# Academich/translation-transformer

Hardware: AMD Instinct MI355X
Metric: reactions/sec (SMILES decoded), greedy speculative (higher is better)
Workload: dtype f32

## Files before the change

include/ttx.h:

```cpp
#ifndef TTX_H
#define TTX_H

#include <stdint.h>

#ifdef __cplusplus
extern "C" {
#endif

#define TTX_ABI_VERSION 4

typedef enum ttx_status {
  TTX_OK = 0,
  TTX_ERR_INVALID = -1,
  TTX_ERR_HIP = -2,
  TTX_ERR_NO_DEVICE = -3,
  TTX_ERR_REFERENCE = -4,
  TTX_ERR_NOMEM = -5,
  TTX_ERR_ROW_REPLAY = -6,
  TTX_ERR_MAX_STEPS = -7
} ttx_status;

typedef struct ttx_config {
  int32_t vocab_size;
  int32_t src_vocab_size;
// ... 490 lines not shown
  int32_t* d_row_of; int32_t* d_slot_batch; int32_t* d_src_acc; int32_t* d_src_state; int32_t* d_tok; int32_t* d_drafts_all;
  int32_t* d_bat_id; int32_t* d_bat_iter; int32_t* d_bat_dl; int32_t* d_bat_grp; int32_t* d_bat_live; int32_t* d_bat_nfin;
  int32_t* d_bat_longest_fin; int32_t* d_bat_longest_cur; int32_t* d_bat_state; int32_t* d_bat_given;
  int64_t* d_cand_next; int32_t* d_len_next; uint8_t* d_fin_next; float* d_logp_next; int32_t* d_parent; int32_t* d_parent_draft;
  int32_t* d_gen; int32_t* d_front; int32_t* d_len; uint8_t* d_active; uint8_t* d_finished; uint8_t* d_live; float* d_logp;
  int32_t* d_per_cand; int32_t* d_drafts32; int32_t* d_cand_dl; int32_t* d_cand_batch; int32_t* d_cache_slot; int32_t* d_cache_slot_parent;
  const int32_t* d_chosen_slot; const int64_t* d_chosen; const float* d_leaf_score; const int32_t* d_leaf_tok; const int32_t* d_leaf_cnt;
  int32_t* d_dev_summary;
  int64_t* d_out; int16_t* d_trace_len; int32_t* d_summary; const int32_t* d_len_all; const int32_t* d_batch_all; const int32_t* d_given_all;
  int32_t* d_src_of; int32_t* d_cand_src_len; int32_t* d_new_slot;
  const int32_t* d_tok_new; const uint8_t* d_valid_new; uint8_t* d_src_valid; const int32_t* d_drafts_new; float* d_memkv;
  const float* d_memkv_new;
  int32_t C, K, N, D0, Ls_cap, max_len, ld, smart, lib_ld, pad, bos, eos, repl, max_steps;
  int32_t T_cap, R, first_row, kv_row, Ls_new;
} ttx_debug_bsp_args;
int ttx_debug_bsp(ttx_session* s, int op, const ttx_debug_bsp_args* a, int64_t* words, void* stream);

int ttx_debug_kvcopy(ttx_session* s, const int32_t* d_rec, int n_copy, const float* d_qkv, int64_t qkv_layer_stride, float* d_kcache,
                     float* d_vcache, int64_t cache_layer_stride, int64_t cache_seq_stride, int N, int D, int d, int B, int Ld,
                     void* stream);

int ttx_debug_kvcopy_split(ttx_session* s, const int32_t* d_rec, int n_copy, const float* d_qkv, int64_t qkv_layer_stride,
                           float* d_kcache, float* d_vcache, int64_t cache_layer_stride, int64_t cache_seq_stride, int N, int D, int d,
                           int B, int Ld, const int32_t* d_pos2, const float* d_qkv_probe, int64_t probe_layer_stride, void* stream);

int ttx_debug_probe_split(ttx_session* s, const int32_t* d_act_idx, const int32_t* d_pred_probe, const int32_t* d_drafts, int B, int N,
                          int D, int n_active, int32_t* d_act2, int32_t* d_pos2, int32_t* result, void* stream);

int ttx_debug_merge_pred(ttx_session* s, const int32_t* d_pos2, const int32_t* d_pred_probe, const int32_t* d_pred2, int32_t* d_pred,
                         int B, int N, int D, int n_active, void* stream);

int ttx_debug_probe_split_select(ttx_session* s, const int32_t* d_act_idx, const int32_t* d_pred_probe, const int32_t* d_drafts, int B,
                                 int N, int D, int n_active, int32_t* d_act2, int32_t* d_pos2, int32_t* d_draft_mask, int32_t* d_row_base,
                                 int32_t* d_row_map, int32_t* result, void* stream);
int ttx_debug_merge_pred_select(ttx_session* s, const int32_t* d_pos2, const int32_t* d_pred_probe, const int32_t* d_pred2,
                                int32_t* d_pred, int B, int N, int D, int n_active, const int32_t* d_row_base,
                                const int32_t* d_draft_mask, void* stream);
int ttx_debug_kvcopy_select(ttx_session* s, const int32_t* d_rec, int n_copy, const float* d_qkv, int64_t qkv_layer_stride,
                            float* d_kcache, float* d_vcache, int64_t cache_layer_stride, int64_t cache_seq_stride, int N, int D, int d,
                            int B, int Ld, const int32_t* d_pos2, const float* d_qkv_probe, int64_t probe_layer_stride,
                            const int32_t* d_row_base, const int32_t* d_draft_mask, void* stream);
int ttx_debug_embed_select(ttx_session* s, const float* d_table, int V, const float* d_pe, int pe_rows, int d, float* d_x,
                           const int32_t* d_act_idx, const int32_t* d_front, const int32_t* d_gen, int gen_ld, const int32_t* d_drafts,
                           int B, int N, int D, int n_active, const int32_t* d_row_map, int m_rows, void* stream);
int ttx_debug_attn_select(ttx_session* s, const float* d_q, int ldq, const float* d_k, const float* d_v, int ldkv, float* d_out, int H,
                          float scale, int Lk, const int32_t* d_tok, int pad, const uint8_t* d_key_pad, const int32_t* d_act_idx,
                          const int32_t* d_front, const int32_t* d_src_of, const int32_t* d_src_len, const float* d_kcache,
                          const float* d_vcache, int64_t cache_seq_stride, const int32_t* d_cache_slot, int gen_ld, int N, int D, int mode,
                          int groups, int n_active, int max_keys, int kernel, int32_t* kernel_id, const int32_t* d_row_base,
                          const int32_t* d_draft_mask, void* stream);

int ttx_pool_last_counters(ttx_session* s, int64_t* counters);

int ttx_attn_staged_key_limit(int head_dim, int q_per_group);

int ttx_debug_attn_kernels_seen(ttx_session* s);

int ttx_debug_attn_probs(ttx_session* s, const float* d_q, int ldq, const float* d_k, int ldkv, const uint8_t* d_key_pad,
                         const int32_t* d_mem_row, const int32_t* d_length, int R, int Rm, int H, int head_dim, int T, int Ls,
                         float scale, float* d_heads, float* d_mean, int32_t* d_align, void* stream);

#ifdef __cplusplus
}
#endif
#endif
```

translation-transformer_amd/_native.py:

```python
from __future__ import annotations

import ctypes as C
import os
import subprocess
from pathlib import Path

PKG_DIR = Path(__file__).resolve().parent
CSRC = PKG_DIR / "csrc"
INCLUDE = PKG_DIR.parent / "include"
LIB_PATH = PKG_DIR / "libttx_hip.so"
UNITS = [CSRC / "ttx_api.hip", CSRC / "ttx_gemm.hip", CSRC / "ttx_attn.hip"]
HEADERS = [CSRC / "ttx_internal.h", CSRC / "ttx_common.hip.h", CSRC / "ttx_loop_kernels.hip.h", CSRC / "ttx_metrics.hip.h",
           CSRC / "ttx_score.hip.h", CSRC / "ttx_alternatives.hip.h", CSRC / "ttx_attn_probs.hip.h", CSRC / "ttx_sample.hip.h", CSRC / "ttx_logq.hip.h", CSRC / "ttx_sbs.hip.h", CSRC / "ttx_sbs_pool.hip.h",
           CSRC / "ttx_proposal.hip.h",
           CSRC / "ttx_select.h", CSRC / "ttx_tokenizer.h", CSRC / "ttx_drive.h", CSRC / "ttx_admit.h", INCLUDE / "ttx.h"]
SOURCES = UNITS + HEADERS
OBJ_DIR = CSRC / "build"

TTX_OK, TTX_ERR_INVALID, TTX_ERR_HIP, TTX_ERR_NO_DEVICE, TTX_ERR_REFERENCE, TTX_ERR_NOMEM = 0, -1, -2, -3, -4, -5
TTX_ERR_ROW_REPLAY = -6
TTX_ERR_MAX_STEPS = -7
TTX_ACT_NONE, TTX_ACT_RELU, TTX_ACT_GELU = 0, 1, 2
ACTIVATIONS = {"relu": TTX_ACT_RELU, "gelu": TTX_ACT_GELU}

# ... 275 lines not shown
                                 C.POINTER(C.c_int32), _VP]),
    "ttx_debug_gemm_act": (C.c_int, [_VP, _VP, _I, _VP, _I, _VP, _VP, _I, _VP, _I, _I, _I, _I, _I, C.c_int64, _I, _I,
                                     C.POINTER(C.c_int32), _VP]),
    "ttx_debug_finish_ln": (C.c_int, [_VP, _VP, _I, C.c_int64, _VP, _VP, _VP, _VP, _VP, _VP, _VP, _VP, _VP, _I, _I, C.c_float, _VP]),
    "ttx_debug_attn": (C.c_int, [_VP, _VP, _I, _VP, _VP, _I, _VP, _I, C.c_float, _I, _I, _VP, _I, _VP, _VP, _VP, _VP, _VP, _VP, _VP, _VP,
                                 C.c_int64, _VP, _I, _I, _I, _I, _I, _I, _I, _I, C.POINTER(C.c_int32), _VP]),
    "ttx_debug_attn_hd": (C.c_int, [_VP, _VP, _I, _VP, _VP, _I, _VP, _I, _I, C.c_float, _I, _I, _VP, _I, _VP, _VP, _VP, _VP, _VP, _VP, _VP,
                                    _VP, C.c_int64, _VP, _I, _I, _I, _I, _I, _I, _I, _I, C.POINTER(C.c_int32), _VP]),
    "ttx_debug_attn_as": (C.c_int, [_VP, _VP, _I, _VP, _VP, _I, _VP, _I, _I, C.c_float, _I, _I, _VP, _I, _VP, _VP, _VP, _VP, _VP, _VP, _VP,
                                    _VP, C.c_int64, _VP, _I, _I, _I, _I, _I, _I, _I, _I, C.POINTER(C.c_int32), _I, _I, _VP]),
    "ttx_debug_argmax": (C.c_int, [_VP, _VP, _I, _VP, _VP, _I, _VP]),
    "ttx_debug_sample": (C.c_int, [_VP, _VP, _I, _VP, _VP, _VP, _VP, _VP, _VP, _I, C.POINTER(SampleParams), _VP]),
    "ttx_debug_sample_step": (C.c_int, [_VP, _VP, _I, _VP, _VP, _VP, _VP, _I, _I, _I, _I, _VP, _VP, C.POINTER(SampleParams), _VP]),
    "ttx_debug_sample_accept": (C.c_int, [_VP, C.POINTER(DebugAcceptArgs), C.POINTER(C.c_int64), _VP]),
    "ttx_debug_sample_step_select": (C.c_int, [_VP, _VP, _I, _VP, _VP, _VP, _VP, _I, _I, _I, _I, _VP, _VP, C.POINTER(SampleParams),
                                              _VP, _I, _VP]),
    "ttx_debug_prefix_drafts": (C.c_int, [_VP, _VP, _VP, _I, _I, _I, _I, _VP, _VP, C.POINTER(DebugPrefix), _I, _I, _I, _VP]),
    "ttx_debug_proposal_drafts": (C.c_int, [_VP, _VP, _VP, _VP, _I, _I, _I, _I, _I, _VP, _VP, C.POINTER(DebugPrefix), _I, _I, _I, _I,
                                            _I, _VP]),
    "ttx_debug_sample_prefix": (C.c_int, [_VP, _VP, _I, _VP, _VP, _VP, _VP, _VP, _VP, _I, C.POINTER(SampleParams),
                                         C.POINTER(DebugPrefix), _VP]),
    "ttx_debug_sample_step_prefix": (C.c_int, [_VP, _VP, _I, _VP, _VP, _VP, _VP, _I, _I, _I, _I, _VP, _VP, C.POINTER(SampleParams),
                                              _VP, _I, C.POINTER(DebugPrefix), _VP]),
    "ttx_debug_sample_accept_pool": (C.c_int, [_VP, C.POINTER(DebugAcceptArgs), C.POINTER(C.c_int64), _VP, _I, _VP]),
    "ttx_debug_pool_fill_sample": (C.c_int, [_VP, C.POINTER(DebugPoolFillArgs), C.POINTER(C.c_int32), _VP]),
    "ttx_debug_embed": (C.c_int, [_VP, _VP, _I, _VP, _I, _I, _VP, _VP, _I, _I, _VP, _VP, _VP, _I, _VP, _I, _I, _I, _I, _I, _VP]),
    "ttx_debug_accept": (C.c_int, [_VP, C.POINTER(DebugAcceptArgs), C.POINTER(C.c_int64), _VP]),
    "ttx_debug_accept_block": (C.c_int, [_VP, C.POINTER(C.c_int32), _I, _VP]),
    "ttx_debug_bs_prep": (C.c_int, [_VP, C.POINTER(DebugBsPrepArgs), _VP]),
    "ttx_debug_bs_list": (C.c_int, [_VP, C.POINTER(DebugBsListArgs), C.POINTER(C.c_int64), _VP]),
    "ttx_debug_bs_hits": (C.c_int, [_VP, C.POINTER(DebugBsHitsArgs), _VP]),
    "ttx_debug_bs_leaves": (C.c_int, [_VP, C.POINTER(DebugBsLeavesArgs), _VP]),
    "ttx_debug_beam_select": (C.c_int, [_VP, C.POINTER(DebugBeamSelectArgs), _VP]),
    "ttx_debug_beam_step": (C.c_int, [_VP, C.POINTER(DebugBeamStepArgs), _VP]),
    "ttx_debug_sbs_step": (C.c_int, [_VP, C.POINTER(DebugSbsStepArgs), _VP]),
    "ttx_debug_sbs_step_ex": (C.c_int, [_VP, C.POINTER(DebugSbsStepArgs), _I, C.c_float, C.POINTER(DebugPrefix), _I, _VP]),
    "ttx_debug_sbs_step_pool": (C.c_int, [_VP, C.POINTER(DebugSbsStepPoolArgs), _I, _I, C.c_float, C.POINTER(DebugPrefix), _VP]),
    "ttx_debug_sbs_pool": (C.c_int, [_VP, _I, C.POINTER(DebugSbsPoolArgs), C.POINTER(C.c_int64), _VP]),
    "ttx_debug_tree_cache": (C.c_int, [_VP, C.POINTER(DebugTreeCacheArgs), _VP]),
    "ttx_debug_bsp": (C.c_int, [_VP, _I, C.POINTER(DebugBspArgs), C.POINTER(C.c_int64), _VP]),
    "ttx_debug_kvcopy": (C.c_int, [_VP, _VP, _I, _VP, C.c_int64, _VP, _VP, C.c_int64, C.c_int64, _I, _I, _I, _I, _I, _VP]),
    "ttx_debug_kvcopy_split": (C.c_int, [_VP, _VP, _I, _VP, C.c_int64, _VP, _VP, C.c_int64, C.c_int64, _I, _I, _I, _I, _I, _VP, _VP,
                                         C.c_int64, _VP]),
    "ttx_debug_probe_split": (C.c_int, [_VP, _VP, _VP, _VP, _I, _I, _I, _I, _VP, _VP, C.POINTER(C.c_int32), _VP]),
    "ttx_debug_merge_pred": (C.c_int, [_VP, _VP, _VP, _VP, _VP, _I, _I, _I, _I, _VP]),
    "ttx_debug_probe_split_select": (C.c_int, [_VP, _VP, _VP, _VP, _I, _I, _I, _I, _VP, _VP, _VP, _VP, _VP, C.POINTER(C.c_int32), _VP]),
    "ttx_debug_merge_pred_select": (C.c_int, [_VP, _VP, _VP, _VP, _VP, _I, _I, _I, _I, _VP, _VP, _VP]),
    "ttx_debug_kvcopy_select": (C.c_int, [_VP, _VP, _I, _VP, C.c_int64, _VP, _VP, C.c_int64, C.c_int64, _I, _I, _I, _I, _I, _VP, _VP,
                                          C.c_int64, _VP, _VP, _VP]),
    "ttx_debug_embed_select": (C.c_int, [_VP, _VP, _I, _VP, _I, _I, _VP, _VP, _VP, _VP, _I, _VP, _I, _I, _I, _I, _VP, _I, _VP]),
    "ttx_debug_attn_select": (C.c_int, [_VP, _VP, _I, _VP, _VP, _I, _VP, _I, C.c_float, _I, _VP, _I, _VP, _VP, _VP, _VP, _VP, _VP, _VP,
                                        C.c_int64, _VP, _I, _I, _I, _I, _I, _I, _I, _I, C.POINTER(C.c_int32), _VP, _VP, _VP]),
    "ttx_pool_last_counters": (C.c_int, [_VP, C.POINTER(C.c_int64)]),
    "ttx_attn_staged_key_limit": (C.c_int, [_I, _I]),
    "ttx_debug_attn_kernels_seen": (C.c_int, [_VP]),
    "ttx_last_kernel_profile": (C.c_int, [_VP, C.POINTER(C.c_double), C.POINTER(C.c_int64), C.POINTER(C.c_double)]),
}

_lib = None


def hipcc_path() -> str:
    for cand in (os.environ.get("HIPCC"), "/opt/rocm/bin/hipcc", "hipcc"):
        if cand and (os.path.isabs(cand) and os.path.exists(cand) or not os.path.isabs(cand)):
            return cand
    return "hipcc"


def needs_build() -> bool:
    if not LIB_PATH.exists():
        return True
    t = LIB_PATH.stat().st_mtime
    return any(src.stat().st_mtime > t for src in SOURCES)


def build(force: bool = False, verbose: bool = False) -> Path:
    if not force and not needs_build():
        return LIB_PATH
    OBJ_DIR.mkdir(exist_ok=True)
    flags = ["--offload-arch=gfx950", "-O3", "-std=c++17", "-fPIC", f"-I{INCLUDE}"] + os.environ.get("TTX_HIPCC_FLAGS", "").split()
    newest_header = max(h.stat().st_mtime for h in HEADERS)
    jobs, objs = [], []
    for unit in UNITS:
        obj = OBJ_DIR / (unit.stem + ".o")
        objs.append(str(obj))
        if not force and obj.exists() and obj.stat().st_mtime > max(unit.stat().st_mtime, newest_header) \
                and not os.environ.get("TTX_HIPCC_FLAGS"):
            continue
        cmd = [hipcc_path(), *flags, "-c", str(unit), "-o", str(obj)]
        if verbose:
            print(" ".join(cmd))
        jobs.append((cmd, subprocess.Popen(cmd)))
    for cmd, proc in jobs:
        if proc.wait() != 0:
            raise subprocess.CalledProcessError(proc.returncode, cmd)
    cmd = [hipcc_path(), "--offload-arch=gfx950", "-shared", "-fPIC", "-o", str(LIB_PATH), *objs]
    if verbose:
        print(" ".join(cmd))
    subprocess.run(cmd, check=True)
    return LIB_PATH


def lib():
    global _lib
    if _lib is not None:
        return _lib
# ... 23 lines not shown
```

translation-transformer_amd/csrc/ttx_admit.h:

```cpp
#pragma once
#include <algorithm>
#include <cstdint>
#include <vector>

namespace ttx {

inline int pool_slot_width(int len_max, int max_positions) {
  const int w = std::min(std::max(192, ((len_max + 63) / 64) * 64), max_positions);
  return std::max(w, std::max(2, len_max));
}

struct PoolShape { int n_jobs, C; };
inline PoolShape pool_shape(int n_sessions, int n_batches, int R_total, int capacity, int small_pool, int max_batch) {
  const int per_pool = std::max(1, std::min(capacity / 2, small_pool));
  const int n_jobs = std::max(1, std::min({n_sessions, n_batches, (R_total + per_pool - 1) / per_pool}));
  return {n_jobs, std::min(capacity, std::max(max_batch, (R_total + n_jobs - 1) / n_jobs))};
}

inline int serial_quota(const int* first, int n_batches, int cursor, int job, int n_jobs) {
  const int rest = first[n_batches] - first[cursor];
  const int target = first[cursor] + (rest + (n_jobs - job) - 1) / (n_jobs - job);
  int end = cursor;
  while (end < n_batches && first[end] < target) ++end;
  return end;
}

struct AdmitState {
  int cursor;
  int free_slots;
  int n_live;
  bool first_fill;
  int job, n_jobs;
  int n_running;
  bool serial;
  int quota_end;
};

inline int plan_admission(const int* first, int n_batches, int C, const AdmitState& a) {
  const int list_end = a.serial ? a.quota_end : n_batches;
  const int min_admit = std::max(1, C / 4);
  if (a.cursor >= list_end) return 0;
  if (a.n_live != 0 && a.free_slots < std::max(min_admit, first[a.cursor + 1] - first[a.cursor])) return 0;
  const int remaining = first[list_end] - first[a.cursor];
  const auto cdiv = [](int x, int y) { return (x + y - 1) / y; };
  int share = std::max(1, cdiv(remaining, std::max(1, a.serial ? 1 : a.n_running)));
  if (!a.serial && a.first_fill && (long long)a.n_jobs * C >= first[n_batches]) share = std::max(1, cdiv(remaining, a.n_jobs - a.job));
  int take = 0, end = a.cursor;
  while (end < list_end) {
    const int sz = first[end + 1] - first[end];
    if (take + sz > a.free_slots || (take > 0 && take + sz > share)) break;
    take += sz;
    ++end;
  }
  return end - a.cursor;
}

constexpr long long ADMIT_ROWS = 16384;
inline int chunk_width(const int32_t* len, int first, int end) {
  int w = 2;
  for (int r = first; r < end; ++r) w = std::max(w, (int)len[r]);
  return w;
}
inline void admit_chunks(const int32_t* len, int n, long long budget, std::vector<int>& ends) {
  ends.clear();
  if (budget > 0 && (long long)n * chunk_width(len, 0, n) >= budget) {
    int first = 0, w = 2;
    for (int r = 0; r < n; ++r) {
      w = std::max(w, (int)len[r]);
      if ((long long)(r + 1 - first) * w >= budget) { ends.push_back(r + 1); first = r + 1; w = 2; }
    }
    if (first < n) {
      const bool merge = !ends.empty() && (long long)(n - first) * chunk_width(len, first, n) * 2 < budget;
      if (merge) ends.back() = n; else ends.push_back(n);
    }
  } else {
    ends.push_back(n);
  }
}

}
```

translation-transformer_amd/csrc/ttx_api.hip:

```cpp
#include "ttx_internal.h"
#include "ttx_admit.h"
#include "ttx_drive.h"
#include "ttx_loop_kernels.hip.h"
#include "ttx_metrics.hip.h"
#include "ttx_score.hip.h"
#include "ttx_alternatives.hip.h"
#include "ttx_attn_probs.hip.h"
#include "ttx_sample.hip.h"
#include "ttx_logq.hip.h"
#include "ttx_sbs.hip.h"
#include "ttx_sbs_pool.hip.h"
#include "ttx_proposal.hip.h"
#include "ttx_tokenizer.h"

#include <algorithm>
#include <chrono>
#include <cmath>
#include <cstdio>
#include <cstdlib>
#include <cstring>
#include <mutex>
#include <type_traits>

using namespace ttx;
// ... 2036 lines not shown
  const int kcap = k.max_len;
  const int matches = ((volatile ProbeInfo*)s->probe_info)->matches;
  if (matches < 0 || matches > k.B) return fail(TTX_ERR_HIP, "slot pool: the probe published a match count outside the pool");
  const int RPS = step_rps(k.N, k.D);
  const long long rows = j.draft_select ? ((volatile ProbeInfo*)s->probe_info)->rows : (long long)matches * RPS;
  if (rows < (long long)matches * (matches ? 1 + k.D : 0) || rows > (long long)matches * RPS)
    return fail(TTX_ERR_HIP, "slot pool: the probe published a row count outside its matches' rows");
  DecState* st2 = s->state2.as<DecState>();
  k.st_ov = st2 + 1; k.act_ov = s->act2.as<int>(); k.pred_ov = s->pred_draft.as<int>();
  if (j.draft_select) { k.row_base = s->row_base.as<int>(); k.draft_mask = s->draft_mask.as<int>(); k.row_map = s->row_map.as<int>(); }
  k.variant = matches ? variant_for_rows(s, rows, true) : 0;
  j.matched_slot_steps += matches; j.skipped_draft_passes += matches ? 0 : 1;
  j.rows_executed += rows; j.drafts_matched += (rows - matches) / k.D;
  const int phase = j.draft_select ? (matches ? 5 : 6) : (matches ? 2 : 3);
  TTX_TRY(graph_replay(s, j.st, s->step_graphs, pool_key(j, k, k.variant, phase), [&]() -> int {
    if (matches) TTX_TRY(run_step(s, j.st, k, kcap));
    MergePredArgs mp{};
    mp.st = s->state.as<DecState>(); mp.pos2 = s->pos2.as<int>(); mp.pred_probe = s->pred_probe.as<int>();
    mp.pred2 = s->pred_draft.as<int>(); mp.pred = s->pred.as<int>(); mp.RPS = RPS;
    mp.row_base = k.row_base; mp.draft_mask = k.draft_mask; mp.D = k.D;
    hipLaunchKernelGGL(k_merge_pred, dim3(cdiv(k.B * RPS, 256)), dim3(256), 0, j.st, mp);
    HIP_TRY(hipGetLastError());
    return launch_accept_and_commit(s, j.st, j.g2, false);
  }));
  j.probe_pending = false;
  ++j.launched;
  return TTX_OK;
}

static int pool_sample_begin(PoolJob& j, const SampleSetup& smp) {
  ttx_session* s = j.s;
  hipLaunchKernelGGL(k_sample_params, dim3(1), dim3(64), 0, j.st, s->smp_prm.as<SampleBlock>(), smp.blk);
  HIP_TRY(hipGetLastError());
  StepCtx& k = j.g.k;
  k.want_sample_step = true;
  k.sample.key = s->smp_key.as<unsigned long long>(); k.sample.sample = s->smp_sample.as<unsigned>();
  k.sample.front = s->front.as<int>(); k.sample.prm = s->smp_prm.as<SampleBlock>();
  j.g.la.sample_rule = 1;
  j.per_src = smp.n; j.d_row_keys = smp.d_row_keys;
  if (smp.tabled()) {
    TTX_TRY(prefix_upload(s, j.st, smp, k.max_len, k.p.pad_token));
    const PrefixTab tab{s->pfx_tok.as<int>(), k.max_len, s->pfx_len.as<int>(), s->pfx_src.as<int>()};
    if (smp.proposed) { k.prop = tab; k.prop_ctx = smp.prop_ctx; }
    else k.sample.pfx = tab;
    k.pfx_draft0 = s->pfx_draft0.as<int>();
  }
  return TTX_OK;
}

static int pool_generate(ttx_session** sessions, int n_sessions, const int64_t* d_src, int R_total, int Ls_all, const int32_t* h_len,
                         int Ls_cap, int capacity, const ttx_gen_params* p, int64_t* d_out, int16_t* d_traj, int32_t* d_fin_step,
                         ttx_gen_stats* stats, void* stream, const SampleSetup* smp) {
  const int per = smp ? smp->n : 1;
  const PoolShape shape = pool_shape(n_sessions, R_total, R_total * per, capacity, 32, per);
  const int n_jobs = shape.n_jobs, C = shape.C;
  std::vector<int> first(R_total + 1);
  for (int r = 0; r <= R_total; ++r) first[r] = r * per;
  std::vector<PoolJob> jobs(n_jobs);
  std::vector<int> chunk_ends;
  std::fill(std::begin(sessions[0]->pool_counters), std::end(sessions[0]->pool_counters), 0LL);
  const bool serial = sessions[0]->profile;
  int cursor = 0;
  const auto start = [&](int i) -> int {
    TTX_TRY(pool_start(jobs[i], sessions[i], sessions[i]->own_stream, C, Ls_cap, p, d_out, d_traj, d_fin_step, smp));
    if (i == 0) sessions[0]->pool_counters[6] = jobs[0].draft_select ? 1 : 0;
    return TTX_OK;
  };
  const auto turn = [&](int i) -> int {
    PoolJob& j = jobs[i];
    ttx_session* s = j.s;
    volatile HostInfo* hi = s->host_info;
    if (j.phase == 1) {
      if (j.probe_pending) {
        if (((volatile ProbeInfo*)s->probe_info)->probes_done < j.probes) return TURN_WAITING;
        TTX_TRY(pool_launch_drafts(j));
        return TURN_PROGRESSED;
      }
      if (j.launched > 0 && hi->steps_done < j.launched) return TURN_WAITING;
      int n_act = (j.launched == 0) ? 0 : hi->n_active;
      if (serial && j.quota_end < 0) j.quota_end = serial_quota(first.data(), R_total, cursor, i, n_jobs);
      int n_running = 0;
      for (const PoolJob& o : jobs) n_running += (o.phase == 1);
      const int take = plan_admission(first.data(), R_total, C, {cursor, C - n_act, n_act, j.launched == 0, i, n_jobs, n_running, serial, j.quota_end});
      if (take > 0) {
        admit_chunks(h_len + cursor, take, j.admit_rows, chunk_ends);
        int r0 = cursor;
        for (const int end : chunk_ends) {
          const int r1 = cursor + end;
          TTX_TRY(pool_admit(j, d_src + (size_t)r0 * Ls_all, Ls_all, r1 - r0, chunk_width(h_len, r0, r1), r0, d_out, d_traj, d_fin_step));
          r0 = r1;
        }
        n_act += first[cursor + take] - first[cursor];
        cursor += take;
      }
      if (n_act == 0) {
        TTX_TRY(enqueue_readback(s, j.st, s->state.p, sizeof(DecState)));
        j.phase = 2;
      } else {
        if (j.launched > (long long)(p->max_len + 2) * (R_total + 1)) return fail(TTX_ERR_HIP, "decode loop failed to terminate");
        TTX_TRY(pool_launch_step(j, n_act));
      }
      return TURN_PROGRESSED;
    }
    if (hipEventQuery(s->ev_done) != hipSuccess) return TURN_IDLE;
    const DecState& hs = *s->host_state;
    if (stats) {
      add_counters(*stats, hs);
      stats->src_tokens_padded += j.src_tokens_padded;
      collect_gemm_profile(s, j.st);
      float ms = 0.f;
      if (hipEventElapsedTime(&ms, s->ev_a, s->ev_c) == hipSuccess) stats->decode_ms += ms;
    }
    if (getenv("TTX_TWO_PHASE_STATS"))
      fprintf(stderr, "[ttx two-phase] pool %d: %d steps, %lld split (%lld without a draft pass), %lld slot-steps probed, %lld matched, "
                      "%lld draft rows executed, %lld drafts matched\n",
              i, j.launched, j.split_steps, j.skipped_draft_passes, j.slot_steps, j.matched_slot_steps,
              j.rows_executed - j.slot_steps - j.unsplit_rows, j.drafts_matched);
    long long* pc = sessions[0]->pool_counters;
    pc[0] += j.launched; pc[1] += j.split_steps; pc[2] += j.slot_steps; pc[3] += j.matched_slot_steps;
    pc[4] += j.drafts_matched; pc[5] += j.rows_executed;
    j.phase = 3;
    if (hs.error == 3) return fail(TTX_ERR_ROW_REPLAY, "a row emitted PAD inside its sequence: decode the batches as given");
    if (hs.error) return fail(TTX_ERR_HIP, "slot pool bookkeeping failed (admitted more rows than free slots)");
    return TURN_FINISHED;
  };
  const int rc = drive_sessions(sessions, n_jobs, serial, stream, start, turn);
  if (stats) stats->status = rc;
  return rc;
}

extern "C" int ttx_greedy_speculative_generate_pool(ttx_session** sessions, int n_sessions, const int64_t* d_src, int R_total,
                                                    int Ls_all, const int32_t* h_len, int capacity, const ttx_gen_params* p,
                                                    int64_t* d_out, int16_t* d_traj, int32_t* d_fin_step, ttx_gen_stats* stats,
                                                    void* stream) {
  if (!sessions || n_sessions <= 0 || !d_src || R_total < 0 || !h_len || capacity <= 0 || capacity > 4096 || !p || !d_out || !d_traj ||
      !d_fin_step)
    return fail(TTX_ERR_INVALID, "bad argument to ttx_greedy_speculative_generate_pool");
  if (R_total == 0) return TTX_OK;
  if (p->max_len > 32000) return fail(TTX_ERR_INVALID, "max_len too large for the int16 trace");
  int len_max = 0;
  for (int i = 0; i < R_total; ++i) len_max = std::max(len_max, (int)h_len[i]);
  if (len_max > Ls_all) return fail(TTX_ERR_INVALID, "row length beyond the source matrix width");
  const int Ls_cap = pool_slot_width(len_max, sessions[0]->m->cfg.max_positions);
  TTX_TRY(gen_validate(sessions[0], d_src, capacity, Ls_cap, p, d_out, false));
  return pool_generate(sessions, n_sessions, d_src, R_total, Ls_all, h_len, Ls_cap, capacity, p, d_out, d_traj, d_fin_step, stats, stream,
                       nullptr);
// ... 2728 lines not shown
static int merge_pred_debug(ttx_session* s, const int32_t* d_pos2, const int32_t* d_pred_probe, const int32_t* d_pred2,
                            int32_t* d_pred, int B, int N, int D, int n_active, const int32_t* d_row_base, const int32_t* d_draft_mask,
                            void* stream) {
  hipStream_t st = reinterpret_cast<hipStream_t>(stream);
  if (!s || !d_pos2 || !d_pred_probe || !d_pred2 || !d_pred) return fail(TTX_ERR_INVALID, "null argument to ttx_debug_merge_pred");
  if (B < 1 || N < 1 || D < 1) return fail(TTX_ERR_INVALID, "ttx_debug_merge_pred: B, N and D must be positive");
  if (n_active < 0 || n_active > B) return fail(TTX_ERR_INVALID, "ttx_debug_merge_pred: n_active must lie in [0, B]");
  HIP_TRY(hipSetDevice(s->m->device));
  HIP_TRY(hipStreamSynchronize(st));
  if (n_active > 0) {
    std::vector<int> pos((size_t)n_active);
    HIP_TRY(hipMemcpy(pos.data(), d_pos2, (size_t)n_active * 4, hipMemcpyDeviceToHost));
    for (int p : pos)
      if (p < -1 || p >= B) return fail(TTX_ERR_INVALID, "ttx_debug_merge_pred: pos2 must lie in [-1, B)");
    if (d_row_base || d_draft_mask) {
      int n_pos = 0, total = 0;
      for (int p : pos) n_pos = std::max(n_pos, p + 1);
      TTX_TRY(dbg_check_select("ttx_debug_merge_pred_select", d_row_base, d_draft_mask, n_pos, N, D, st, nullptr, &total));
    }
  }
  DecState* dst = nullptr;
  TTX_TRY(dbg_state_with(st, n_active, 0, &dst));
  MergePredArgs mp{};
  mp.st = dst; mp.pos2 = d_pos2; mp.pred_probe = d_pred_probe; mp.pred2 = d_pred2; mp.pred = d_pred; mp.RPS = step_rps(N, D);
  mp.row_base = d_row_base; mp.draft_mask = d_draft_mask; mp.D = D;
  hipLaunchKernelGGL(k_merge_pred, dim3(cdiv(B * mp.RPS, 256)), dim3(256), 0, st, mp);
  hipError_t err = hipGetLastError();
  const hipError_t esync = hipStreamSynchronize(st);
  (void)hipFree(dst);
  HIP_TRY(err);
  HIP_TRY(esync);
  return TTX_OK;
}

extern "C" int ttx_debug_merge_pred(ttx_session* s, const int32_t* d_pos2, const int32_t* d_pred_probe, const int32_t* d_pred2,
                                    int32_t* d_pred, int B, int N, int D, int n_active, void* stream) {
  return merge_pred_debug(s, d_pos2, d_pred_probe, d_pred2, d_pred, B, N, D, n_active, nullptr, nullptr, stream);
}

extern "C" int ttx_debug_merge_pred_select(ttx_session* s, const int32_t* d_pos2, const int32_t* d_pred_probe, const int32_t* d_pred2,
                                           int32_t* d_pred, int B, int N, int D, int n_active, const int32_t* d_row_base,
                                           const int32_t* d_draft_mask, void* stream) {
  if ((d_row_base != nullptr) != (d_draft_mask != nullptr))
    return fail(TTX_ERR_INVALID, "ttx_debug_merge_pred_select: row_base and draft_mask come together");
  return merge_pred_debug(s, d_pos2, d_pred_probe, d_pred2, d_pred, B, N, D, n_active, d_row_base, d_draft_mask, stream);
}

extern "C" int ttx_pool_last_counters(ttx_session* s, int64_t* counters) {
  if (!s || !counters) return fail(TTX_ERR_INVALID, "null argument to ttx_pool_last_counters");
  for (int i = 0; i < 7; ++i) counters[i] = s->pool_counters[i];
  return TTX_OK;
}

extern "C" int ttx_attn_staged_key_limit(int head_dim, int q_per_group) { return attn_staged_key_limit(head_dim, q_per_group); }

extern "C" int ttx_debug_attn_kernels_seen(ttx_session* s) {
  if (!s) return fail(TTX_ERR_INVALID, "null session");
  return (int)s->attn_kernels_seen;
}

extern "C" int ttx_last_kernel_profile(ttx_session* s, double* gemm_ms, int64_t* gemm_launches, double* empty_pair_ms) {
  if (!s) return fail(TTX_ERR_INVALID, "null session");
  if (gemm_ms) *gemm_ms = s->prof_ms;
  if (gemm_launches) *gemm_launches = s->prof_launches;
  s->prof_ms = 0;
  s->prof_launches = 0;
  if (empty_pair_ms) *empty_pair_ms = s->prof_empty_pair_ms < 0 ? 0.0 : s->prof_empty_pair_ms;
  return TTX_OK;
}
```

translation-transformer_amd/csrc/ttx_internal.h:

```cpp
#pragma once
#include "ttx.h"
#include "ttx_common.hip.h"

#include <map>
#include <set>
#include <string>
#include <utility>
#include <vector>

namespace ttx {
struct BeamHost;
struct BeamPoolHost;
}

struct LayerW {
  size_t sa_in_w, sa_in_b, sa_out_w, sa_out_b;
  size_t ca_in_w, ca_in_b, ca_out_w, ca_out_b;
  size_t l1_w, l1_b, l2_w, l2_b;
  size_t n1_w, n1_b, n2_w, n2_b, n3_w, n3_b;
};

struct ttx_model {
  ttx_config cfg;
  int device;
// ... 52 lines not shown
  X(ev_logits) X(ev_pred) X(ev_nll)                                                                                              \
   \
                                                                                                      \
  X(sc_src_of) X(am_length)                                                                                                                   \
                                    \
  X(lq_tok)                                                                                                                      \
                                                                                                                       \
  X(drafts) X(gen) X(front) X(act_idx) X(rec) X(pred) X(state) X(kcache) X(vcache) X(src32) X(outbuf) X(haspad) X(traj)           \
  X(fin_step)                                                                                                                    \
                                                                                            \
  X(rstep) X(row_of) X(src_len) X(new_slot) X(pool_io) X(memkv_new) X(valid_new) X(drafts_new)                                    \
       \
            \
  X(qkv_probe) X(pred_probe) X(pred_draft) X(act2) X(pos2) X(state2)                                                             \
         \
  X(draft_mask) X(row_base) X(row_map)                                                                                           \
                           \
  X(accept_blk)                                                                                                                  \
                                        \
  X(snap_logits) X(snap_act) X(snap_front) X(snap_gen) X(snap_state)                                                             \
  X(leaf_score) X(leaf_tok) X(leaf_cnt) X(beam_summary)                                                                          \
                                                                                               \
  X(bs_cand_next) X(bs_len_next) X(bs_fin_next) X(bs_logp_next) X(bs_len) X(bs_fin) X(bs_active) X(bs_logp) X(bs_per_cand)        \
  X(bs_best_n) X(bs_best_slot) X(bs_chosen) X(bs_parent) X(bs_parent_draft) X(bs_mark) X(bs_drafts_src) X(bs_cnt) X(bs_hit)       \
                                                                                 \
  X(t_prev_len) X(t_slot_of) X(t_src_of)                                                                                         \
                                            \
  X(bp_row_of) X(bp_batch) X(bp_cand) X(bp_cand_len) X(bp_tok) X(bp_new_slot) X(bp_io) X(bp_grp) X(bp_src_acc) X(bp_enc_qkv)            \
   \
                     \
  X(smp_key) X(smp_sample) X(smp_done) X(smp_src_of) X(smp_prm) X(smp_drafts)                                                     \
   \
       \
  X(pfx_tok) X(pfx_len_src) X(pfx_len) X(pfx_src) X(pfx_draft0)                                                                  \
    \
  X(sbs_g) X(sbs_g_next)                                                                                                         \
   \
                                                                                          \
  X(sbp_slot) X(sbp_len) X(sbp_io)
#define TTX_DECLARE_BUF(name) Buf name;
#define TTX_REGISTER_BUF(name) all.push_back(&name);

#ifndef TTX_BIG_MIN_TILES
#define TTX_BIG_MIN_TILES 400
#endif
struct ttx_session {
  ttx_model* m;
  std::vector<Buf*> all;
  TTX_SESSION_BUFS(TTX_DECLARE_BUF)
  Buf tk[2], tv[2];
  int snap_B = 0, snap_rps = 0, snap_gen_ld = 0, snap_step = 0;
  ttx::ProbeInfo* probe_info = nullptr;
  long long pool_counters[7] = {};
  ttx::BeamHost* beam_host = nullptr;
  ttx::BeamPoolHost* bp_host = nullptr;
  ttx::HostInfo* host_info = nullptr;
  hipStream_t own_stream = nullptr;
  uint64_t alloc_generation = 0;
  uint64_t graphs_generation = 0;
  bool dead = false;
  bool use_graphs = true;
  GraphCache step_graphs{512};
  GraphCache iter_graphs{256};
  hipEvent_t ev_done = nullptr;
  void drop_graphs() { step_graphs.clear(); iter_graphs.clear(); }
  void graphs_current() { if (graphs_generation != alloc_generation) { drop_graphs(); graphs_generation = alloc_generation; } }
  ttx::DecState* host_state = nullptr;
  bool attr_attn2[2][8] = {};
  bool attr_select = false, attr_step = false, attr_topk = false, attr_pool_select = false, attr_sbs_step = false;
  bool attr_sbs_step_masked[5] = {};
  bool attr_sbs_step_pool = false, attr_sbs_step_pool_masked[5] = {};
  bool attr_attn_probs[8] = {};
  int qkv_small_rows = 800;
  int small_rows = 2000;
  int ffn2_slab_rows = 5600;
  int big_min_tiles = TTX_BIG_MIN_TILES;
  int last_gemm_kernel = 0, last_gemm_big_min_tiles = 0;
  int attn_split = -1;
  int attn_row = -1;
  bool accept_spread = true;
  bool attn_fallback = false;
  int attn_force = 0;
  int attn_sel_N = 0, attn_sel_D = 0;
  int last_attn_kernel = 0;
  unsigned attn_kernels_seen = 0;
  bool profile = false;
  std::vector<std::pair<hipEvent_t, hipEvent_t>> ev_pool;
  size_t ev_used = 0;
  double prof_ms = 0;
  double prof_empty_pair_ms = -1;
  long long prof_launches = 0;
  bool host_timing = false;
  double host_launch_us = 0;
  long long host_captures = 0;
  double host_capture_us = 0;
  long long host_launches = 0;
  hipEvent_t ev_a = nullptr, ev_b = nullptr, ev_c = nullptr;
  ttx_session() {
    TTX_SESSION_BUFS(TTX_REGISTER_BUF)
    for (Buf* b : {&tk[0], &tk[1], &tv[0], &tv[1]}) all.push_back(b);
    for (Buf* b : all) b->owner_gen = &alloc_generation;
  }
};

namespace ttx {

// ... 45 lines not shown
```

translation-transformer_amd/decoding.py:

```python
from __future__ import annotations

import ctypes as C
import os
from typing import NamedTuple

import numpy as np
import torch

from . import _native as N
from .model import AttentionMaps, HypothesisScores, NativeTransformer, ProposalScores


def _need_native(model) -> NativeTransformer:
    if not isinstance(model, NativeTransformer):
        raise TypeError("the native generators run on a NativeTransformer (no eager/PyTorch fallback exists)")
    return model


class _ScoresHypotheses:

    def _pad_eos(self) -> tuple:
        return self.pad_token, self.eos_token

    def score(self, src: torch.Tensor, pred: torch.Tensor, **kw) -> HypothesisScores:
# ... 121 lines not shown
            return []
        if reorder:
            try:
                if pool is None:
                    pool = True
                return self._generate_reordered(batches, in_flight, group_size, on_error, pool)
            except N.TtxError as e:
                if e.code != N.TTX_ERR_ROW_REPLAY:
                    raise
        srcs = [b.to(m.device, torch.int64).contiguous() for b in batches]
        for b in srcs:
            m.check_tokens(b)
        outs = [torch.empty((s.shape[0], 1, self.max_len), dtype=torch.int64, device=m.device) for s in srcs]
        n = len(srcs)
        pool = m.session_pool(max(1, min(in_flight, n)))
        sess = (C.c_void_p * len(pool))(*[p.value for p in pool])
        src_p = (C.c_void_p * n)(*[s.data_ptr() for s in srcs])
        out_p = (C.c_void_p * n)(*[o.data_ptr() for o in outs])
        Bs = (C.c_int * n)(*[s.shape[0] for s in srcs])
        Ls = (C.c_int * n)(*[s.shape[1] for s in srcs])
        p = N.GenParams(self.max_len, self.draft_len, self.n_drafts, self.pad_token, self.bos_token, self.eos_token,
                        self.replace_token, 0)
        stats = (N.GenStats * n)()
        rc = m._lib.ttx_greedy_speculative_generate_many(sess, len(pool), n, src_p, Bs, Ls, C.byref(p), out_p, stats, m._stream())
        if not (rc == N.TTX_ERR_REFERENCE and on_error == "skip"):
            N.check(rc)
        t = self.stats_total
        for i, st in enumerate(stats):
            if st.status != N.TTX_OK:
                if st.status != N.TTX_ERR_REFERENCE:
                    N.check(int(st.status))
                outs[i] = None
                self.last_failed_batches.append(i)
                continue
            self.model_calls_num += int(st.model_calls)
            self.last_batch_counters[i] = {"model_calls_num": int(st.model_calls)}
            for k in ("accepted_tokens", "produced_tokens", "verified_positions", "kv_prefix_positions", "src_positions",
                      "encode_ms", "decode_ms"):
                t[k] += getattr(st, k)
            t["src_tokens_padded"] += srcs[i].shape[0] * srcs[i].shape[1]
            t["batches"] += 1
        return outs

    def _generate_reordered(self, batches: list, in_flight: int, group_size: int | None, on_error: str = "raise",
                            pool: bool = True) -> list:
        from .scheduling import plan_row_groups, replay_batch
        m = self.model
        L, T = self.max_len, self.max_len + 1
        srcs = [b.to(m.device, torch.int64) for b in batches]
        sizes = [int(s.shape[0]) for s in srcs]
        R = sum(sizes)
        if pool:
            gsz, pool_sessions = _slot_pool_plan(R, in_flight, group_size)
        else:
            gsz = int(group_size or min(256, max(max(sizes), -(-R // max(1, in_flight)))))
        self.last_group_size = gsz
        Lmax = max(int(s.shape[1]) for s in srcs)
        allsrc = torch.full((R, Lmax), self.pad_token, dtype=torch.int64, device=m.device)
        r0 = 0
        for s in srcs:
            allsrc[r0:r0 + s.shape[0], :s.shape[1]] = s
            r0 += s.shape[0]
        m.check_tokens(allsrc)
        pos = torch.arange(1, Lmax + 1, device=m.device)
        lengths = ((allsrc != self.pad_token) * pos).amax(dim=1)
        order, groups = plan_row_groups(lengths.cpu().numpy(), gsz)
        order_t = torch.from_numpy(order).to(m.device)
        sorted_src = allsrc[order_t]
        sorted_len = lengths[order_t].cpu().numpy()
        out_sorted = torch.empty((R, L), dtype=torch.int64, device=m.device)
        traj_sorted = torch.empty((R, T), dtype=torch.int16, device=m.device)
        fin_sorted = torch.empty((R,), dtype=torch.int32, device=m.device)
        p = N.GenParams(L, self.draft_len, self.n_drafts, self.pad_token, self.bos_token, self.eos_token, self.replace_token, 0)
        if pool:
            sessions = m.session_pool(pool_sessions)
            sess = (C.c_void_p * len(sessions))(*[q.value for q in sessions])
            width = max(2, int(sorted_len.max()))
            src_mat = sorted_src[:, :width].contiguous() if width <= sorted_src.shape[1] else torch.nn.functional.pad(
                sorted_src, (0, width - sorted_src.shape[1]), value=self.pad_token).contiguous()
            h_len = (C.c_int32 * R)(*[int(x) for x in sorted_len])
            one = N.GenStats()
            N.check(m._lib.ttx_greedy_speculative_generate_pool(sess, len(sessions), src_mat.data_ptr(), R, width, h_len, gsz,
                                                                C.byref(p), out_sorted.data_ptr(), traj_sorted.data_ptr(),
                                                                fin_sorted.data_ptr(), C.byref(one), m._stream()))
            stats, gsrc = [one], [src_mat]
        else:
            gsrc = [sorted_src[g, :max(2, int(sorted_len[g].max()))].contiguous() for g in groups]
            n = len(gsrc)
            sessions = m.session_pool(max(1, min(in_flight, n)))
            sess = (C.c_void_p * len(sessions))(*[q.value for q in sessions])
            src_p = (C.c_void_p * n)(*[s.data_ptr() for s in gsrc])
            out_p = (C.c_void_p * n)(*[out_sorted[g].data_ptr() for g in groups])
            traj_p = (C.c_void_p * n)(*[traj_sorted[g].data_ptr() for g in groups])
            fin_p = (C.c_void_p * n)(*[fin_sorted[g].data_ptr() for g in groups])
            Bs = (C.c_int * n)(*[s.shape[0] for s in gsrc])
            Ls = (C.c_int * n)(*[s.shape[1] for s in gsrc])
            stats = (N.GenStats * n)()
            N.check(m._lib.ttx_greedy_speculative_generate_rows(sess, len(sessions), n, src_p, Bs, Ls, C.byref(p), out_p, traj_p, fin_p,
                                                                stats, m._stream()))
        inv = torch.empty_like(order_t)
        inv[order_t] = torch.arange(R, device=m.device)
        out_rows = out_sorted[inv]
        traj = traj_sorted[inv].cpu().numpy()
        fin = fin_sorted[inv].cpu().numpy()
        keep = torch.zeros(R, dtype=torch.bool)
        t = self.stats_total
        failed = None
        r0 = 0
        for bi, B in enumerate(sizes):
            rep = replay_batch(traj[r0:r0 + B], fin[r0:r0 + B], L, self.draft_len, self.n_drafts)
            if rep.error:
                if on_error == "skip":
                    self.last_failed_batches.append(bi)
                    r0 += B
                    continue
                failed = bi
                break
            keep[r0:r0 + B] = torch.from_numpy(rep.finished)
            self.model_calls_num += rep.model_calls
            self.last_batch_counters[bi] = {"model_calls_num": rep.model_calls}
            t["accepted_tokens"] += rep.accepted_tokens
            t["produced_tokens"] += rep.produced_tokens
            t["verified_positions"] += rep.verified_positions
            t["kv_prefix_positions"] += rep.kv_prefix_positions
            t["src_positions"] += rep.rows_iterations * int(srcs[bi].shape[1])
            t["src_tokens_padded"] += B * int(srcs[bi].shape[1])
            t["batches"] += 1
            r0 += B
        for st in stats:
            t["encode_ms"] += st.encode_ms
            t["decode_ms"] += st.decode_ms
        dv = t.setdefault("device", {"model_calls": 0, "accepted_tokens": 0, "produced_tokens": 0, "verified_positions": 0,
                                     "kv_prefix_positions": 0, "src_positions": 0, "src_tokens_padded": 0, "batches": 0})
        for st, gs in zip(stats, gsrc):
            for k in ("model_calls", "accepted_tokens", "produced_tokens", "verified_positions", "kv_prefix_positions",
                      "src_positions"):
                dv[k] += int(getattr(st, k))
            dv["src_tokens_padded"] += int(st.src_tokens_padded) if pool else int(gs.numel())
            dv["batches"] += 1
        t["device_model_calls"] = dv["model_calls"]
        if failed is not None:
            raise N.ReferenceError_(f"batch {failed}: a row finished at a width beyond max_len: shape mismatch in the reference "
                                    "(speculative_decoding.py:158)")
        out_rows = torch.where(keep.to(m.device)[:, None], out_rows, torch.full_like(out_rows, self.pad_token))
        outs, r0 = [], 0
        skipped = set(self.last_failed_batches)
        for bi, B in enumerate(sizes):
            outs.append(None if bi in skipped else out_rows[r0:r0 + B].unsqueeze(1).contiguous())
            r0 += B
        return outs


class TranslationInferenceGreedy(_ScoresHypotheses):

    def __init__(self, model, max_len: int, pad_token: int, bos_token: int, eos_token: int) -> None:
        self.model = _need_native(model)
        self.max_len = max_len
# ... 703 lines not shown
```

translation-transformer_amd/model.py:

```python
from __future__ import annotations

import ctypes as C
import os
import math
from typing import NamedTuple

import numpy as np
import torch

from . import _native as N


def reference_pe_table(emb: int, max_len: int = 5000) -> torch.Tensor:
    pe = torch.zeros(max_len, emb)
    position = torch.arange(0, max_len, dtype=torch.float).unsqueeze(1)
    div_term = torch.exp(torch.arange(0, emb, 2).float() * (-math.log(10000.0) / emb))
    pe[:, 0::2] = torch.sin(position * div_term)
    pe[:, 1::2] = torch.cos(position * div_term)
    return torch.vstack((torch.zeros(1, emb), pe)).contiguous()


def _strip(state: dict) -> dict:
    if any(k.startswith("model.") for k in state):
        return {k[len("model."):]: v for k, v in state.items() if k.startswith("model.")}
# ... 531 lines not shown
                                n: int, d: int, n_active: int, row_base: torch.Tensor | None, draft_mask: torch.Tensor | None) -> None:
        N.check(self._lib.ttx_debug_merge_pred_select(self._session, pos2.data_ptr(), pred_probe.data_ptr(), pred2.data_ptr(),
                                                      pred.data_ptr(), int(B), int(n), int(d), int(n_active), self._ptr(row_base),
                                                      self._ptr(draft_mask), self._stream()))

    def debug_kvcopy_select(self, rec: torch.Tensor, n_copy: int, qkv: torch.Tensor, kcache: torch.Tensor, vcache: torch.Tensor,
                            n: int, d: int, width: int, B: int, pos2: torch.Tensor | None, qkv_probe: torch.Tensor | None,
                            row_base: torch.Tensor | None, draft_mask: torch.Tensor | None) -> None:
        assert kcache.stride() == vcache.stride()
        N.check(self._lib.ttx_debug_kvcopy_select(self._session, rec.data_ptr(), int(n_copy), qkv.data_ptr(), int(qkv.stride(0)),
                                                  kcache.data_ptr(), vcache.data_ptr(), int(kcache.stride(0)), int(kcache.stride(1)),
                                                  int(n), int(d), int(width), int(B), int(qkv.shape[0]), self._ptr(pos2),
                                                  self._ptr(qkv_probe), 0 if qkv_probe is None else int(qkv_probe.stride(0)),
                                                  self._ptr(row_base), self._ptr(draft_mask), self._stream()))

    def debug_embed_select(self, table: torch.Tensor, pe: torch.Tensor, x: torch.Tensor, act_idx: torch.Tensor, front: torch.Tensor,
                           gen: torch.Tensor, drafts: torch.Tensor, B: int, n: int, d: int, n_active: int,
                           row_map: torch.Tensor | None, m_rows: int) -> None:
        N.check(self._lib.ttx_debug_embed_select(self._session, table.data_ptr(), int(table.shape[0]), pe.data_ptr(), int(pe.shape[0]),
                                                 int(table.shape[1]), x.data_ptr(), act_idx.data_ptr(), front.data_ptr(),
                                                 gen.data_ptr(), int(gen.stride(0)), drafts.data_ptr(), int(B), int(n), int(d),
                                                 int(n_active), self._ptr(row_map), int(m_rows), self._stream()))

    def debug_attn_select(self, mode: int, q: torch.Tensor, k: torch.Tensor, v: torch.Tensor, out: torch.Tensor, heads: int,
                          scale: float, groups: int, max_keys: int, row_base: torch.Tensor | None, draft_mask: torch.Tensor | None,
                          Lk: int = 0, tok: torch.Tensor | None = None, pad: int = 0, key_pad: torch.Tensor | None = None,
                          act_idx: torch.Tensor | None = None, front: torch.Tensor | None = None, src_of: torch.Tensor | None = None,
                          src_len: torch.Tensor | None = None, kcache: torch.Tensor | None = None, vcache: torch.Tensor | None = None,
                          cache_seq_stride: int = 0, cache_slot: torch.Tensor | None = None, gen_ld: int = 0, n: int = 1, d: int = 0,
                          n_active: int = 0, kernel: int = 0, **unused) -> int:
        kid = C.c_int32(0)
        assert k.stride(0) == v.stride(0)
        N.check(self._lib.ttx_debug_attn_select(self._session, q.data_ptr(), q.stride(0), k.data_ptr(), v.data_ptr(), k.stride(0),
                                                out.data_ptr(), int(heads), float(scale), int(Lk), self._ptr(tok), int(pad),
                                                self._ptr(key_pad), self._ptr(act_idx), self._ptr(front), self._ptr(src_of),
                                                self._ptr(src_len), self._ptr(kcache), self._ptr(vcache), int(cache_seq_stride),
                                                self._ptr(cache_slot), int(gen_ld), int(n), int(d), int(mode), int(groups),
                                                int(n_active), int(max_keys), int(kernel), C.byref(kid), self._ptr(row_base),
                                                self._ptr(draft_mask), self._stream()))
        return int(kid.value)

    def attn_kernels_seen(self, session=None) -> set:
        mask = int(self._lib.ttx_debug_attn_kernels_seen(self._session if session is None else session))
        if mask < 0:
            N.check(mask)
        return {k for k in range(1, 32) if mask >> k & 1}

    POOL_COUNTERS = ("steps", "split_steps", "slot_steps_probed", "slots_matched", "drafts_matched", "rows_executed", "draft_select")

    def pool_last_counters(self, session=None) -> dict:
        words = (C.c_int64 * 7)()
        N.check(self._lib.ttx_pool_last_counters(self._session if session is None else session, words))
        return dict(zip(self.POOL_COUNTERS, (int(v) for v in words)))

    @staticmethod
    def attn_staged_key_limit(head_dim: int, q_per_group: int) -> int:
        return int(N.lib().ttx_attn_staged_key_limit(int(head_dim), int(q_per_group)))

    def close(self) -> None:
        if getattr(self, "_score_session", None):
            self._lib.ttx_session_destroy(self._score_session)
            self._score_session = None
        for extra in getattr(self, "_pool", [])[1:]:
            self._lib.ttx_session_destroy(extra)
        self._pool = None
        if getattr(self, "_session", None):
            self._lib.ttx_session_destroy(self._session)
            self._session = None
        if getattr(self, "_model", None):
            self._lib.ttx_model_destroy(self._model)
            self._model = None

    def __del__(self):
        try:
            self.close()
        except Exception:
            pass

    def _tokens(self, t: torch.Tensor) -> torch.Tensor:
        return t.to(self.device, torch.int64).contiguous()

    def check_tokens(self, t: torch.Tensor, vocab: int | None = None) -> None:
        if t.numel() == 0:
            return
        lo, hi = int(t.min()), int(t.max())
        if lo < 0 or hi >= (vocab or self.src_vocab_size):
            raise IndexError("index out of range in self")

    def encode_src(self, src: torch.Tensor, src_pad_mask: torch.Tensor | None = None) -> torch.Tensor:
        src = self._tokens(src)
        self.check_tokens(src)
        B, Ls = src.shape
        mem = torch.empty((B, Ls, self.emb_dim), dtype=torch.float32, device=self.device)
        N.check(self._lib.ttx_encode_src(self._session, src.data_ptr(), B, Ls, mem.data_ptr(), self._stream()))
        return mem

    def decode_tgt(self, tgt: torch.Tensor, memory: torch.Tensor, memory_pad_mask: torch.Tensor,
                   memory_row: torch.Tensor | None = None) -> torch.Tensor:
        tgt = self._tokens(tgt)
        R, Lt = tgt.shape
        memory = memory.to(self.device, torch.float32).contiguous()
        Rm, Ls, _ = memory.shape
        pad = memory_pad_mask.to(self.device, torch.uint8).contiguous()
        row_ptr = None
        if memory_row is not None:
            memory_row = memory_row.to(self.device, torch.int32).contiguous()
# ... 366 lines not shown
```

Baseline: 23880.

## Add dedicated head pool job that decodes the first rows alongside bulk pools

Adds a separate head session that takes the first H rows, by default three quarters of the capacity, in a single admission. The remaining rows are spread over the bulk pool jobs, and the Python planner adds one extra pool session when the head plan applies. The aim is to start work on the leading rows straight away and keep the device busy while bulk jobs run, which should improve overlap and load balance. It costs one more concurrent session, changes admission accounting, and adds layout introspection APIs.

```diff
diff --git a/include/ttx.h b/include/ttx.h
--- a/include/ttx.h
+++ b/include/ttx.h
@@ -566,6 +566,10 @@
 
 int ttx_pool_last_counters(ttx_session* s, int64_t* counters);
 
+int ttx_pool_last_layout(ttx_session* s, int32_t* words);
+
+int ttx_head_pool_rows(int n_sessions, int rows_total, int capacity);
+
 int ttx_attn_staged_key_limit(int head_dim, int q_per_group);
 
 int ttx_debug_attn_kernels_seen(ttx_session* s);
diff --git a/translation-transformer_amd/_native.py b/translation-transformer_amd/_native.py
--- a/translation-transformer_amd/_native.py
+++ b/translation-transformer_amd/_native.py
@@ -351,6 +351,8 @@
     "ttx_debug_attn_select": (C.c_int, [_VP, _VP, _I, _VP, _VP, _I, _VP, _I, C.c_float, _I, _VP, _I, _VP, _VP, _VP, _VP, _VP, _VP, _VP,
                                         C.c_int64, _VP, _I, _I, _I, _I, _I, _I, _I, _I, C.POINTER(C.c_int32), _VP, _VP, _VP]),
     "ttx_pool_last_counters": (C.c_int, [_VP, C.POINTER(C.c_int64)]),
+    "ttx_pool_last_layout": (C.c_int, [_VP, C.POINTER(C.c_int32)]),
+    "ttx_head_pool_rows": (C.c_int, [_I, _I, _I]),
     "ttx_attn_staged_key_limit": (C.c_int, [_I, _I]),
     "ttx_debug_attn_kernels_seen": (C.c_int, [_VP]),
     "ttx_last_kernel_profile": (C.c_int, [_VP, C.POINTER(C.c_double), C.POINTER(C.c_int64), C.POINTER(C.c_double)]),
diff --git a/translation-transformer_amd/csrc/ttx_admit.h b/translation-transformer_amd/csrc/ttx_admit.h
--- a/translation-transformer_amd/csrc/ttx_admit.h
+++ b/translation-transformer_amd/csrc/ttx_admit.h
@@ -15,6 +15,17 @@
   const int per_pool = std::max(1, std::min(capacity / 2, small_pool));
   const int n_jobs = std::max(1, std::min({n_sessions, n_batches, (R_total + per_pool - 1) / per_pool}));
   return {n_jobs, std::min(capacity, std::max(max_batch, (R_total + n_jobs - 1) / n_jobs))};
+}
+
+constexpr int HEAD_POOL_NUM = 3, HEAD_POOL_DEN = 4;
+struct HeadPoolPlan { int head_units, head_capacity; };
+inline HeadPoolPlan head_pool_plan(int n_sessions, int n_units, int rows_total, int capacity, int per, int request) {
+  if (n_sessions < 2 || per > 1 || request == 0 || capacity <= 0) return {0, 0};
+  if ((long long)rows_total < 2LL * (n_sessions - 1) * capacity) return {0, 0};
+  if (request < 0 && n_sessions < 3) return {0, 0};
+  const int units = std::min({request < 0 ? (int)((long long)capacity * HEAD_POOL_NUM / HEAD_POOL_DEN) : request, capacity, n_units - 1});
+  if (units < 1) return {0, 0};
+  return {units, units};
 }
 
 inline int serial_quota(const int* first, int n_batches, int cursor, int job, int n_jobs) {
@@ -55,6 +66,15 @@
   return end - a.cursor;
 }
 
+struct Admission { int from, n; };
+inline Admission head_pool_admission(const int* first, int n_units, int H, int C, const AdmitState& a) {
+  const int hb = H > 0 ? 1 : 0;
+  if (a.job < hb) return {0, a.first_fill ? H : 0};
+  AdmitState b = a;
+  b.cursor = a.cursor - H; b.job = a.job - hb; b.n_jobs = a.n_jobs - hb;
+  return {a.cursor, plan_admission(first, n_units - H, C, b)};
+}
+
 constexpr long long ADMIT_ROWS = 16384;
 inline int chunk_width(const int32_t* len, int first, int end) {
   int w = 2;
diff --git a/translation-transformer_amd/csrc/ttx_api.hip b/translation-transformer_amd/csrc/ttx_api.hip
--- a/translation-transformer_amd/csrc/ttx_api.hip
+++ b/translation-transformer_amd/csrc/ttx_api.hip
@@ -2112,16 +2112,22 @@
                          int Ls_cap, int capacity, const ttx_gen_params* p, int64_t* d_out, int16_t* d_traj, int32_t* d_fin_step,
                          ttx_gen_stats* stats, void* stream, const SampleSetup* smp) {
   const int per = smp ? smp->n : 1;
-  const PoolShape shape = pool_shape(n_sessions, R_total, R_total * per, capacity, 32, per);
-  const int n_jobs = shape.n_jobs, C = shape.C;
+  const char* head_env = getenv("TTX_HEAD_POOL");
+  const HeadPoolPlan head = head_pool_plan(n_sessions, R_total, R_total * per, capacity, per, head_env ? std::max(0, atoi(head_env)) : -1);
+  const int H = head.head_units, hb = H > 0 ? 1 : 0, R_bulk = R_total - H;
+  const PoolShape shape = pool_shape(n_sessions - hb, R_bulk, R_bulk * per, capacity, 32, per);
+  const int n_jobs = hb + shape.n_jobs, n_bulk = shape.n_jobs;
   std::vector<int> first(R_total + 1);
   for (int r = 0; r <= R_total; ++r) first[r] = r * per;
   std::vector<PoolJob> jobs(n_jobs);
   std::vector<int> chunk_ends;
   std::fill(std::begin(sessions[0]->pool_counters), std::end(sessions[0]->pool_counters), 0LL);
+  const int layout[4] = {n_jobs, H, head.head_capacity, shape.C};
+  std::copy(layout, layout + 4, sessions[0]->pool_layout);
   const bool serial = sessions[0]->profile;
-  int cursor = 0;
+  int cursor = H;
   const auto start = [&](int i) -> int {
+    const int C = i < hb ? head.head_capacity : shape.C;
     TTX_TRY(pool_start(jobs[i], sessions[i], sessions[i]->own_stream, C, Ls_cap, p, d_out, d_traj, d_fin_step, smp));
     if (i == 0) sessions[0]->pool_counters[6] = jobs[0].draft_select ? 1 : 0;
     return TTX_OK;
@@ -2138,20 +2144,22 @@
       }
       if (j.launched > 0 && hi->steps_done < j.launched) return TURN_WAITING;
       int n_act = (j.launched == 0) ? 0 : hi->n_active;
-      if (serial && j.quota_end < 0) j.quota_end = serial_quota(first.data(), R_total, cursor, i, n_jobs);
+      const int C = j.C;
+      if (serial && i >= hb && j.quota_end < 0) j.quota_end = serial_quota(first.data(), R_bulk, cursor - H, i - hb, n_bulk);
       int n_running = 0;
-      for (const PoolJob& o : jobs) n_running += (o.phase == 1);
-      const int take = plan_admission(first.data(), R_total, C, {cursor, C - n_act, n_act, j.launched == 0, i, n_jobs, n_running, serial, j.quota_end});
+      for (int o = hb; o < n_jobs; ++o) n_running += (jobs[o].phase == 1);
+      const Admission adm = head_pool_admission(first.data(), R_total, H, C, {cursor, C - n_act, n_act, j.launched == 0, i, n_jobs, n_running, serial, j.quota_end});
+      const int from = adm.from, take = adm.n;
       if (take > 0) {
-        admit_chunks(h_len + cursor, take, j.admit_rows, chunk_ends);
-        int r0 = cursor;
+        admit_chunks(h_len + from, take, j.admit_rows, chunk_ends);
+        int r0 = from;
         for (const int end : chunk_ends) {
-          const int r1 = cursor + end;
+          const int r1 = from + end;
           TTX_TRY(pool_admit(j, d_src + (size_t)r0 * Ls_all, Ls_all, r1 - r0, chunk_width(h_len, r0, r1), r0, d_out, d_traj, d_fin_step));
           r0 = r1;
         }
-        n_act += first[cursor + take] - first[cursor];
-        cursor += take;
+        n_act += first[from + take] - first[from];
+        if (i >= hb) cursor += take;
       }
       if (n_act == 0) {
         TTX_TRY(enqueue_readback(s, j.st, s->state.p, sizeof(DecState)));
@@ -4986,6 +4994,17 @@
   return TTX_OK;
 }
 
+extern "C" int ttx_pool_last_layout(ttx_session* s, int32_t* words) {
+  if (!s || !words) return fail(TTX_ERR_INVALID, "null argument to ttx_pool_last_layout");
+  for (int i = 0; i < 4; ++i) words[i] = s->pool_layout[i];
+  return TTX_OK;
+}
+
+extern "C" int ttx_head_pool_rows(int n_sessions, int rows_total, int capacity) {
+  const char* e = getenv("TTX_HEAD_POOL");
+  return head_pool_plan(n_sessions, rows_total, rows_total, capacity, 1, e ? std::max(0, atoi(e)) : -1).head_units;
+}
+
 extern "C" int ttx_attn_staged_key_limit(int head_dim, int q_per_group) { return attn_staged_key_limit(head_dim, q_per_group); }
 
 extern "C" int ttx_debug_attn_kernels_seen(ttx_session* s) {
diff --git a/translation-transformer_amd/csrc/ttx_internal.h b/translation-transformer_amd/csrc/ttx_internal.h
--- a/translation-transformer_amd/csrc/ttx_internal.h
+++ b/translation-transformer_amd/csrc/ttx_internal.h
@@ -128,6 +128,7 @@
   int snap_B = 0, snap_rps = 0, snap_gen_ld = 0, snap_step = 0;
   ttx::ProbeInfo* probe_info = nullptr;
   long long pool_counters[7] = {};
+  int pool_layout[4] = {};
   ttx::BeamHost* beam_host = nullptr;
   ttx::BeamPoolHost* bp_host = nullptr;
   ttx::HostInfo* host_info = nullptr;
diff --git a/translation-transformer_amd/decoding.py b/translation-transformer_amd/decoding.py
--- a/translation-transformer_amd/decoding.py
+++ b/translation-transformer_amd/decoding.py
@@ -197,6 +197,9 @@
         R = sum(sizes)
         if pool:
             gsz, pool_sessions = _slot_pool_plan(R, in_flight, group_size)
+            default_layout = not (group_size or os.environ.get("TTX_POOL_CAPACITY") or os.environ.get("TTX_POOL_SESSIONS"))
+            if default_layout and in_flight > pool_sessions and m._lib.ttx_head_pool_rows(pool_sessions + 1, R, gsz) > 0:
+                pool_sessions += 1
         else:
             gsz = int(group_size or min(256, max(max(sizes), -(-R // max(1, in_flight)))))
         self.last_group_size = gsz
@@ -248,6 +251,7 @@
         out_rows = out_sorted[inv]
         traj = traj_sorted[inv].cpu().numpy()
         fin = fin_sorted[inv].cpu().numpy()
+        self.last_fin_step = fin
         keep = torch.zeros(R, dtype=torch.bool)
         t = self.stats_total
         failed = None
diff --git a/translation-transformer_amd/model.py b/translation-transformer_amd/model.py
--- a/translation-transformer_amd/model.py
+++ b/translation-transformer_amd/model.py
@@ -607,6 +607,13 @@
         words = (C.c_int64 * 7)()
         N.check(self._lib.ttx_pool_last_counters(self._session if session is None else session, words))
         return dict(zip(self.POOL_COUNTERS, (int(v) for v in words)))
+
+    POOL_LAYOUT = ("jobs", "head_rows", "head_capacity", "bulk_capacity")
+
+    def pool_last_layout(self, session=None) -> dict:
+        words = (C.c_int32 * 4)()
+        N.check(self._lib.ttx_pool_last_layout(self._session if session is None else session, words))
+        return dict(zip(self.POOL_LAYOUT, (int(v) for v in words)))
 
     @staticmethod
     def attn_staged_key_limit(head_dim: int, q_per_group: int) -> int:
```

Result: slower. 22530 (-5.7%).
